# lppllppl920/EndoscopyDepthEstimation-Pytorch

Measured on AMD Instinct MI355X. Metric: train frame-pairs/sec at 256x320 bs=8, higher is better.
Workload: dtype f32

## Files before the change

### endoscopydepthestimation-pytorch_amd/_lib.py

```python

import ctypes
import os

import torch

_HERE = os.path.dirname(os.path.abspath(__file__))
LIB_PATH = os.environ.get("ENDO_HIP_LIB") or os.path.join(_HERE, "lib", "libendo_hip.so")

_P = ctypes.c_void_p
_I = ctypes.c_int
_F = ctypes.c_float
_L = ctypes.c_int64

SIGNATURES = {
    "endo_abi_version": (_I, []),
    "endo_error_string": (ctypes.c_char_p, [_I]),
    "endo_depth_scale_fwd": (_I, [_P, _P, _P, _P, _P, _P, _I, _I, _F, _P]),
    "endo_depth_scale_bwd": (_I, [_P, _P, _P, _P, _P, _P, _P, _I, _I, _F, _P]),
    "endo_flow_from_depth_fwd": (_I, [_P, _P, _P, _P, _P, _P, _I, _I, _I, _P]),
    "endo_flow_from_depth_bwd": (_I, [_P, _P, _P, _P, _P, _P, _P, _I, _I, _I, _P]),
    "endo_depth_warp_fwd": (_I, [_P, _P, _P, _P, _P, _P, _P, _P, _I, _I, _I, _F, _P]),
    "endo_depth_warp_bwd": (_I, [_P, _P, _P, _P, _P, _P, _P, _P, _P, _I, _I, _I, _F, _P]),
    "endo_depth_warp_fwd_tiled": (_I, [_P, _P, _P, _P, _P, _P, _P, _P, _I, _I, _I, _F, _I, _I, _P]),
    "endo_depth_warp_bwd_tiled": (_I, [_P, _P, _P, _P, _P, _P, _P, _P, _P, _I, _I, _I, _F, _I, _I, _P]),
# ... 26 lines not shown
    "endo_net16h_fwd": (_I, [_P, _P, _P, _P, _P, _P, _I, _P]),
    "endo_net16_bwd_workspace_bytes": (_L, [_P]),
    "endo_net16h_bwd_workspace_bytes": (_L, [_P]),
    "endo_net16_set_wgrad_overlap": (_I, [_P, _I]),
    "endo_net16h_set_wgrad_overlap": (_I, [_P, _I]),
    "endo_net16_offset": (_L, [_P, _I, _I]),
    "endo_net16h_offset": (_L, [_P, _I, _I]),
    "endo_net16_bwd": (_I, [_P, _P, _P, _P, _P, _P, _I, _P]),
    "endo_net16h_bwd": (_I, [_P, _P, _P, _P, _P, _P, _I, _P]),
    "endo_mask_mul": (_I, [_P, _P, _P, _I, _I, _I, _P]),
    "endo_net_create": (_I, [ctypes.POINTER(_P), _I, _I, _I]),
    "endo_net_create_grouped": (_I, [ctypes.POINTER(_P), _I, _I, _I, _I]),
    "endo_net_groups": (_I, [_P]),
    "endo_net_set_option": (_I, [_P, _I, _I]),
    "endo_net_get_option": (_I, [_P, _I]),
    "endo_net_group_stride": (_L, [_P]),
    "endo_net_destroy": (None, [_P]),
    "endo_net_param_floats": (_L, []),
    "endo_net_bn_floats": (_L, []),
    "endo_net_tape_floats": (_L, [_P]),
    "endo_net_gradws_floats": (_L, [_P]),
    "endo_net_param_offset": (_L, [_I]),
    "endo_net_bn_offset": (_L, [_I, _I]),
    "endo_net_level_channels": (_I, [_I]),
    "endo_net_act_offset": (_L, [_P, _I]),
    "endo_net_tape_offset": (_L, [_P, _I, _I]),
    "endo_net_fwd": (_I, [_P, _P, _P, _P, _P, _P, _I, _P]),
    "endo_net_bwd": (_I, [_P, _P, _P, _P, _P, _P, _P, _I, _P]),
    "endo_sgd_clip_step": (_I, [_P, _P, _P, _P, _L, _F, _F, _F, _F, _I, _P, _P]),
    "endo_sparse_scatter": (_I, [_P, _I, _P, _P, _P, _P, _P, _I, _I, _I, _F, _P, _P, _P, _P, _P, _P]),
# ... 70 lines not shown
```

### endoscopydepthestimation-pytorch_amd/csrc/net.hip

```cpp
#include <new>
#include <vector>

#include "dgrad_kernels.h"
#include "dgrad_block_kernels.h"
#include "dgrad_newmap_kernels.h"
#include "td_dgrad_kernels.h"
#include "td_fwd_kernels.h"
#include "wgrad_taps_kernels.h"
#include "wgrad1x1_kernels.h"
#include "wgrad_nsplit_kernels.h"
#include "wgrad_x3_kernels.h"
#include "wgrad_f34_kernels.h"
#include "wgrad_subpix_kernels.h"
#include "wino_fwd_kernels.h"
#include "wino4_fwd_kernels.h"
#include "dgrad_wino_kernels.h"
#include "dgrad_wino3_kernels.h"


namespace endo {

int run_dgrad_wino3_nl4(const DgradBlockParams& p, const float* const* u, hipStream_t stream);
bool dgrad_wino3p_applies(const DgradBlockParams& p);
int run_dgrad_wino3p_nl4(const DgradBlockParams& p, const float* const* u, int blocks, double* fw_parts, int* blocks_used, hipStream_t stream);

constexpr int kGrowth = 12;
constexpr int kLayers = 4;
constexpr int kFirst = 48;
constexpr int kLevels = 5;
// ... 102 lines not shown

struct endo_net {
    int n, h, w;
    int groups;
    int64_t gs;
    struct Level { int h, w, t; int64_t plane; int64_t act, grad; int64_t sums; int64_t pq; } lv[kLevels + 1];
    int64_t pre_off;
    int64_t saved_off;
    int64_t idx_off[kLevels];
    int64_t sums_off;
    int64_t sums_bytes;
    int64_t tape_floats;
    int64_t partial_off;
    int64_t wino_off;
    int64_t wino4_off;
    int64_t pq_off;
    int64_t pq_floats;
    int64_t scratch_off;
    int64_t scratch_bytes;
    int64_t slot_stride;
    int64_t wg_scratch_off;
    int64_t tuw_scratch_off;
    int64_t wd_off;
    int64_t gplane_off;
    int64_t bias_parts_off;
    int64_t fw_parts_off;
    int64_t bias_parts_floats;
    int64_t gradws_floats;
    hipStream_t wstream;
    hipEvent_t ev_fork, ev_join;
    int opt[ENDO_OPT_COUNT];
};

namespace endo {


constexpr int kBiasPartChannels = 2048;
constexpr int kBiasPartLaunches = 64;
constexpr int kFwPartBlocks = 512;
struct BiasReduceTable {
    int n;
    struct Entry { const float* parts; float* bias; int count; int nparts; } e[kBiasPartLaunches];
};
struct BiasParts {
    BiasReduceTable table;
    int64_t used;
// ... 144 lines not shown
            if (training) {
                const double mean = a.saved[j][go + 2 * c], rstd = a.saved[j][go + 2 * c + 1];
                const double scale = a.gamma[j][c] * rstd;
                const double k = scale * rstd * s2 / count;
                dp += static_cast<double>(static_cast<float>(-k));
                dq += static_cast<double>(static_cast<float>(-scale * s1 / count + k * mean));
            }
        }
        if (training) {
            pq_p[c] += static_cast<float>(dp);
            pq_q[c] += static_cast<float>(dq);
        }
    }
}

__global__ void tu_phase_weights_kernel(const float* __restrict__ w, int cout, int cin, float* __restrict__ out) {
    constexpr int kPhW = 2 * 12 * 16 + 16;
    const int total = 2 * cin * 2 * 12 * 16;
    for (int i = blockIdx.x * blockDim.x + threadIdx.x; i < total; i += gridDim.x * blockDim.x) {
        const int lane16 = i & 15;
        const int slot = (i >> 4) % 12;
        const int t = (i / (16 * 12)) & 1;
        const int ci = (i / (16 * 12 * 2)) % cin;
        const int a = i / (16 * 12 * 2 * cin);
        int ctap, tile;
        if (slot < 3) { ctap = 0; tile = slot; } else if (slot < 9) { ctap = 1; tile = slot - 3; } else { ctap = 2; tile = slot - 9 + 3; }
        const int b = tile / 3, co = (tile % 3) * 16 + lane16;
        float v = 0.f;
        if (co < cout) {
            const float* src = w + (static_cast<int64_t>(co) * cin + ci) * 9;
            const int ky0 = a == 0 ? (t == 0 ? 0 : 1) : (t == 0 ? 0 : 2), ky1 = a == 0 ? (t == 0 ? 0 : 2) : (t == 0 ? 1 : 2);
            int kx0, kx1;
            if (b == 0) { kx0 = ctap == 0 ? 0 : 1; kx1 = ctap == 0 ? 0 : 2; }
            else { kx0 = ctap == 1 ? 0 : 2; kx1 = ctap == 1 ? 1 : 2; }
            for (int ky = ky0; ky <= ky1; ++ky)
                for (int kx = kx0; kx <= kx1; ++kx) v += src[ky * 3 + kx];
        }
        out[(static_cast<int64_t>(a) * cin + ci) * kPhW + (t * 12 + slot) * 16 + lane16] = v;
    }
}

__global__ void tu_subpix_dgrad_weights_kernel(const float* __restrict__ w, int cout, int cin, float* __restrict__ out) {
    const int pitch = 4 * cin + 16;
    const int total = 4 * cout * 4 * cin;
    for (int i = blockIdx.x * blockDim.x + threadIdx.x; i < total; i += gridDim.x * blockDim.x) {
        const int ci = i % cin;
        const int tap = (i / cin) & 3;
        const int co = (i / (4 * cin)) % cout;
        const int ph = i / (4 * cin * cout);
        const int alpha = ph >> 1, beta = ph & 1, tyi = tap >> 1, txi = tap & 1;
        const int ky0 = alpha == 0 ? (tyi == 0 ? 1 : 0) : (tyi == 0 ? 2 : 0), ky1 = alpha == 0 ? (tyi == 0 ? 2 : 0) : (tyi == 0 ? 2 : 1);
        const int kx0 = beta == 0 ? (txi == 0 ? 1 : 0) : (txi == 0 ? 2 : 0), kx1 = beta == 0 ? (txi == 0 ? 2 : 0) : (txi == 0 ? 2 : 1);
        const float* src = w + (static_cast<int64_t>(co) * cin + ci) * 9;
        float v = 0.f;
// ... 118 lines not shown
        const float t = static_cast<float>(scratch[0] + scratch[1] + scratch[2] + scratch[3]);
        if (c < cin) atomicAdd(gw + c, t); else atomicAdd(gb, t);
    }
}

__global__ void __launch_bounds__(64) final_w_reduce_kernel(const double* __restrict__ parts, int nblocks, int count, float* __restrict__ gw) {
    const int c = blockIdx.x;
    double t = 0.0;
    for (int b = threadIdx.x; b < nblocks; b += 64) t += parts[static_cast<int64_t>(b) * count + c];
    t = wave_sum(t);
    if (threadIdx.x == 0) atomicAdd(gw + c, static_cast<float>(t));
}

constexpr int kBlocks = 2 * kLevels + 1, kDense = kBlocks * kLayers;

enum class DenseFwd { Wino4, Wino2_32x16, Wino2_32x8, SplitK, Direct32x8, Direct16x8, DirectAuto };
struct FwdPlan {
    struct Dense {
        DenseFwd form;
        int stages;
        int ksplit;
        bool chunk_weights;
    } dense[kDense];
    bool bf16;
    bool wino4_weights;
    bool fuse_final;
    bool td_persistent[kLevels];
    bool tu_subpix[kLevels];
};

enum class NewMap { Bf16, Persistent, Vec16, Dword };
// ... 102 lines not shown
static double conv_flops(const endo_net* net, int level, int cin, int cout, int ks) {
    return 2.0 * net->n * net->groups * net->lv[level].plane * cin * cout * ks * ks;
}

static void default_options(int (&opt)[ENDO_OPT_COUNT]) {
    opt[ENDO_OPT_WINO_FWD] = 5;
    opt[ENDO_OPT_WINO_DGRAD] = 3;
    opt[ENDO_OPT_DGRAD_VEC] = 2;
    opt[ENDO_OPT_WINO_MIN_TILES] = 1024;
    opt[ENDO_OPT_MFMA_BF16] = 0;
    opt[ENDO_OPT_WGRAD_OVERLAP] = 1;
    opt[ENDO_OPT_MFMA_X3] = 0;
    opt[ENDO_OPT_WGRAD_F34] = 1;
    opt[ENDO_OPT_FINAL_VIRTUAL] = 1;
    opt[ENDO_OPT_TD_PERSIST] = 3;
}
static int bf16_mask(const int* opt) { const int v = opt[ENDO_OPT_MFMA_BF16]; return v == 1 ? 7 : (v >> 1); }

struct DenseBlock { int level, ic0, c0; const BnP* bn; const ConvP* cv; bool base_overwrite; };
static DenseBlock dense_block(int b) {
    const Table& tb = table();
    if (b < kLevels) return {b, 48, down_in(b), tb.down_bn[b], tb.down_conv[b], false};
    if (b == kLevels) return {kLevels, 0, 288, tb.bott_bn, tb.bott_conv, true};
    const int i = b - kLevels - 1, l = kLevels - 1 - i;
    return {l, 0, 96 + down_in(l), tb.up_bn[i], tb.up_conv[i], l > 0};
}
static long tile_count(const Ctx& c, int level, int tx, int ty) {
    const auto& lv = c.net->lv[level];
    return static_cast<long>((lv.w + tx - 1) / tx) * ((lv.h + ty - 1) / ty) * c.nt();
}
// ... 18 lines not shown
    const ConvP& cv = table().td_conv[level];
    const int next = level + 1;
    const int oc0 = next < kLevels ? 48 : 0;
    ConvParams p{};
    fill_grid(c, p, level);
    fill_in(c, p, c.act(level), level, 48, cv.cin);
    fill_bn_in(c, p, b, level, 48);
    p.wgt = c.params + cv.w; p.bias = c.params + cv.b; p.w_cout = cv.cout; p.w_cin = cv.cin;
    fill_out(c, p, c.act(next), next, oc0, cv.cout);
    p.out_idx = c.idx(level);
    p.idx_ns = static_cast<int64_t>(cv.cout) * c.net->lv[next].plane;
    p.out_sums = c.out_sums(next, oc0);
    return p;
}

static FwdPlan plan_fwd(const Ctx& c) {
    const int* opt = c.net->opt;
    const int mode = opt[ENDO_OPT_WINO_FWD];
    const long min_tiles = opt[ENDO_OPT_WINO_MIN_TILES];
    FwdPlan pl{};
    pl.bf16 = (bf16_mask(opt) & 2) != 0;
    pl.wino4_weights = !pl.bf16 && mode == 5;
    for (int b = 0; b < kBlocks; ++b) {
        const DenseBlock k = dense_block(b);
        const long t64x16 = tile_count(c, k.level, 64, 16), t32x16 = tile_count(c, k.level, 32, 16), t32x8 = tile_count(c, k.level, 32, 8);
        const long t16x16 = tile_count(c, k.level, 16, 16), t16x8 = tile_count(c, k.level, 16, 8);
        const bool big = t32x16 >= min_tiles, small = t32x8 >= (min_tiles * 3) / 4;
        const bool wino4_tiles = mode == 5 && !pl.bf16 && 2 * t64x16 >= min_tiles;
        const bool wino2_tiles = mode != 0 && !pl.bf16 && (big || small);
        for (int j = 0; j < kLayers; ++j) {
            FwdPlan::Dense& d = pl.dense[b * kLayers + j];
            const int nchunks = (k.cv[j].cin + 15) / 16;
            d.chunk_weights = !pl.bf16 && !wino4_tiles && !wino2_tiles;
            d.stages = mode == 4 ? 4 : (mode == 3 ? 3 : 2);
            if (wino4_tiles && wino4_fwd_ok(dense_fwd_params(c, k, j, DenseFwd::Wino4))) {
                d.form = DenseFwd::Wino4;
            } else if (wino2_tiles && wino_fwd_ok(dense_fwd_params(c, k, j, DenseFwd::Wino2_32x16))) {
                d.form = big ? DenseFwd::Wino2_32x16 : DenseFwd::Wino2_32x8;
            } else if (t32x16 < 512 && t16x16 < 384 && t16x8 < 512 && nchunks >= 4) {
                int want = static_cast<int>(((t16x8 < 256 ? 512 : 768) + t16x8 - 1) / t16x8);
                if (want > nchunks) want = nchunks;
                const int per = (nchunks + want - 1) / want;
                d.form = DenseFwd::SplitK;
                d.ksplit = (nchunks + per - 1) / per;
            } else {
                d.form = (t32x16 < 1024 && t32x8 >= 1024) ? DenseFwd::Direct32x8
                       : (t32x16 < 1024 && t16x8 >= 768) ? DenseFwd::Direct16x8 : DenseFwd::DirectAuto;
            }
        }
    }
    pl.fuse_final = opt[ENDO_OPT_FINAL_VIRTUAL] && pl.dense[kDense - 1].form == DenseFwd::Wino4;
    for (int l = 0; l < kLevels; ++l) {
        pl.td_persistent[l] = (opt[ENDO_OPT_TD_PERSIST] & 2) && !pl.bf16 && c.training && td_fwd_ok(td_fwd_params(c, l));
        const ConvP& tu = table().tu_conv[kLevels - 1 - l];
        pl.tu_subpix[l] = c.net->lv[l + 1].w % 4 == 0 && tu.cout == kNew && tu.cin % 4 == 0;
    }
    return pl;
}

// ... 22 lines not shown
            p.split_stride = static_cast<int64_t>(c.net->n) * cv.cout * lv.plane;
            p.out = partial; p.out_ns = static_cast<int64_t>(cv.cout) * lv.plane;
            p.bias = nullptr; p.out_sums = nullptr;
            p.wgt_chunks = chunk_weights;
            int rc = bf16 ? launch_conv_dma<3, 16, 1, IN_BNRELU, EPI_FWD, 1, 2, 2, 1, 1>(p, c.stream)
                          : launch_conv_dma<3, 16, 1, IN_BNRELU, EPI_FWD, 1, 2, 2, 1>(p, c.stream);
            if (rc) return rc;
            int bx = static_cast<int>((lv.plane + 255) / 256);
            bx = bx > 8 ? 8 : bx;
            finalize_partial_kernel<<<dim3(bx, cv.cout, c.nt()), 256, 0, c.stream>>>(
                partial, p.split_stride, d.ksplit, p.out_ns, static_cast<int>(lv.plane), c.params + cv.b, c.act(k.level) + oc0 * lv.plane,
                lv.t * lv.plane, c.out_sums(k.level, oc0), c.net->n, c.net->gs);
            ENDO_LAUNCH_CHECK();
            return 0;
        }
        case DenseFwd::Direct32x8:
            return bf16 ? launch_conv_dma<3, 4, 1, IN_BNRELU, EPI_FWD, 2, 4, 2, 1, 1>(p, c.stream) : launch_conv_dma<3, 4, 1, IN_BNRELU, EPI_FWD, 2, 4, 2, 1>(p, c.stream);
        case DenseFwd::Direct16x8:
            return bf16 ? launch_conv_dma<3, 8, 1, IN_BNRELU, EPI_FWD, 1, 2, 2, 1, 1>(p, c.stream) : launch_conv_dma<3, 8, 1, IN_BNRELU, EPI_FWD, 1, 2, 2, 1>(p, c.stream);
        case DenseFwd::DirectAuto:
            if (bf16) return launch_conv_dma_auto<3, 4, 1, IN_BNRELU, EPI_FWD, 8, 2, 1, 1>(p, c.stream);
            p.wgt_chunks = chunk_weights;
            return launch_conv_dma_auto<3, 4, 1, IN_BNRELU, EPI_FWD, 8, 2, 1>(p, c.stream);
    }
    return ENDO_E_BADARG;
}

static int td_fwd(const Ctx& c, int level) {
    const ConvP& cv = table().td_conv[level];
    const ConvParams p = td_fwd_params(c, level);
    ProfScope prof(kProfConv1x1Pool, c.stream, conv_flops(c.net, level, cv.cin, cv.cout, 1),
                   4.0 * c.nt() * c.net->lv[level].plane * (cv.cin + cv.cout / 4.0));
    if (c.fwd->td_persistent[level]) return launch_td_fwd(p, device_cu_count(), c.stream);
    if (c.fwd->bf16) return launch_conv_dma_auto<1, 8, 3, IN_BNRELU, EPI_FWD_POOL, 4, 2, 1, 1>(p, c.stream);
    return launch_conv_dma_auto<1, 8, 3, IN_BNRELU, EPI_FWD_POOL, 4>(p, c.stream);
}

static int tu_fwd(const Ctx& c, int level, int src_level, int src_c0, const ConvP& cv) {
    ProfScope prof(kProfConv3x3Up, c.stream, conv_flops(c.net, level, cv.cin, cv.cout, 3),
                   4.0 * c.nt() * c.net->lv[level].plane * (cv.cin / 4.0 + cv.cout));
    if (c.fwd->tu_subpix[level]) {
        float* w3 = c.tape + c.net->partial_off;
        tu_phase_weights_kernel<<<(2 * cv.cin * 384 + 255) / 256, 256, 0, c.stream>>>(c.params + cv.w, cv.cout, cv.cin, w3);
        ENDO_LAUNCH_CHECK();
        ConvParams p{};
        fill_grid(c, p, src_level);
        fill_in(c, p, c.act(src_level), src_level, src_c0, cv.cin);
        p.wgt = w3; p.w_cout = 2 * cv.cout; p.w_cin = cv.cin;
        p.bias = c.params + cv.b;
        fill_out(c, p, c.act(level), level, 0, cv.cout);
        p.out_sums = c.out_sums(level, 0);
        return launch_conv_dma_vec<3, 4, 6, IN_PLAIN, EPI_FWD, 2, 4, 2, 1, 4, 0, 0, 2>(p, c.stream);
    }
    ConvParams p{};
    fill_grid(c, p, level);
    fill_in(c, p, c.act(src_level), src_level, src_c0, cv.cin);
    p.wgt = c.params + cv.w; p.bias = c.params + cv.b; p.w_cout = cv.cout; p.w_cin = cv.cin;
    fill_out(c, p, c.act(level), level, 0, cv.cout);
    p.out_sums = c.out_sums(level, 0);
// ... 452 lines not shown

static int64_t align_up(int64_t v, int64_t a) { return (v + a - 1) / a * a; }

}

extern "C" int endo_net_create_grouped(endo_net** out, int n, int h, int w, int groups) {
    if (!out || n <= 0 || h <= 0 || w <= 0 || groups <= 0) return ENDO_E_BADARG;
    if (groups > kMaxGroups) return ENDO_E_UNSUPPORTED;
    if ((h % 32) != 0 || (w % 32) != 0) return ENDO_E_UNSUPPORTED;
    const Table& tb = table();
    endo_net* net = new (std::nothrow) endo_net();
    if (!net) return ENDO_E_BADARG;
    net->n = n; net->h = h; net->w = w; net->groups = groups;
    net->wstream = nullptr; net->ev_fork = nullptr; net->ev_join = nullptr;
    default_options(net->opt);
    int64_t off = 0, sums = 0, pq = 0;
    for (int l = 0; l <= kLevels; ++l) {
        auto& lv = net->lv[l];
        lv.h = h >> l; lv.w = w >> l; lv.t = level_channels(l);
        lv.plane = static_cast<int64_t>(lv.h) * lv.w;
        lv.act = off; lv.grad = off;
        off += align_up(static_cast<int64_t>(n) * lv.t * lv.plane, 64);
        lv.sums = sums; sums += 2 * lv.t;
        lv.pq = pq; pq += lv.t;
    }
    const int64_t acts = off;
    net->pre_off = off; off += align_up(static_cast<int64_t>(n) * h * w, 64);
    net->saved_off = off; off += align_up(2 * tb.bn_width_total, 64);
    int64_t byte_off = off * 4;
    for (int l = 0; l < kLevels; ++l) {
        net->idx_off[l] = byte_off;
        byte_off += align_up(static_cast<int64_t>(n) * (down_in(l) + kNew) * net->lv[l + 1].plane, 256);
    }
    net->sums_off = byte_off;
    net->sums_bytes = sums * 8;
    byte_off += align_up(net->sums_bytes, 256);
    net->partial_off = byte_off / 4;
    byte_off += static_cast<int64_t>(kGrowth) * 163840 * 4;
    net->wino_off = byte_off / 4;
    byte_off += align_up(tb.wino_floats * 4, 256);
    net->wino4_off = byte_off / 4;
    byte_off += align_up(tb.wino4_floats * 4, 256);
    net->tape_floats = byte_off / 4;
    net->pq_off = acts;
    net->pq_floats = 2 * pq;
    net->scratch_off = align_up((acts + net->pq_floats) * 4, 256);
    net->slot_stride = align_up(tb.bn_width_total * 2, 32);
    net->scratch_bytes = net->slot_stride * 8 * kBnSlots;
    net->wg_scratch_off = (net->scratch_off + align_up(net->scratch_bytes, 256)) / 4;
    net->tuw_scratch_off = net->wg_scratch_off + std::max(std::max(kNsScratchFloats, kSpScratchFloats), 4 * kF34ScratchFloats);
    net->wd_off = align_up(net->tuw_scratch_off + 4 * kNew * (4 * kNew + 16), 64);
    net->gplane_off = align_up(net->wd_off + tb.wino_dgrad_floats, 64);
    net->bias_parts_off = net->gplane_off + align_up(static_cast<int64_t>(n) * h * w, 64);
    net->bias_parts_floats = static_cast<int64_t>(kBiasPartChannels) * n * groups * 32;
    {
        int launches = 1, channels = tb.first.cout;
        for (int l = 0; l < kLevels; ++l) {
// ... 24 lines not shown
    return net->opt[option_id];
}

extern "C" void endo_net_destroy(endo_net* net) {
    if (!net) return;
    if (net->ev_fork) (void)hipEventDestroy(net->ev_fork);
    if (net->ev_join) (void)hipEventDestroy(net->ev_join);
    if (net->wstream) (void)hipStreamDestroy(net->wstream);
    delete net;
}
extern "C" int64_t endo_net_param_floats(void) { return table().param_floats; }
extern "C" int64_t endo_net_bn_floats(void) { return table().bn_floats; }
extern "C" int64_t endo_net_tape_floats(const endo_net* net) { return !net ? 0 : (net->groups > 1 ? net->groups * net->gs : net->tape_floats); }
extern "C" int64_t endo_net_gradws_floats(const endo_net* net) { return !net ? 0 : (net->groups > 1 ? net->groups * net->gs : net->gradws_floats); }
extern "C" int endo_net_groups(const endo_net* net) { return net ? net->groups : 0; }
extern "C" int64_t endo_net_group_stride(const endo_net* net) { return net ? net->gs : 0; }
extern "C" int64_t endo_net_param_offset(int index) {
    const Table& tb = table();
    if (index < 0 || index >= static_cast<int>(tb.param_offsets.size())) return -1;
    return tb.param_offsets[index];
}
extern "C" int64_t endo_net_bn_offset(int bn_index, int which) {
    const Table& tb = table();
    if (bn_index < 0 || bn_index >= static_cast<int>(tb.bn_order.size()) || which < 0 || which > 1) return -1;
    return tb.bn_order[bn_index]->run + which * tb.bn_order[bn_index]->c;
}
extern "C" int endo_net_level_channels(int level) { return (level < 0 || level > kLevels) ? -1 : level_channels(level); }
extern "C" int64_t endo_net_act_offset(const endo_net* net, int level) { return (!net || level < 0 || level > kLevels) ? -1 : net->lv[level].act; }

extern "C" int64_t endo_net_tape_offset(const endo_net* net, int what, int index) {
// ... 8 lines not shown
            if (index < 0 || index >= kLevels) return -1;
            return net->idx_off[index];
        default: return -1;
    }
}

extern "C" int endo_net_fwd(endo_net* net, const float* params, float* bn_running, const float* x, float* out, float* tape,
                            int training, void* stream_) {
    if (!net || !params || !bn_running || !x || !out || !tape) return ENDO_E_BADARG;
    const Table& tb = table();
    Ctx c{net, params, bn_running, tape, nullptr, nullptr, training, static_cast<hipStream_t>(stream_)};
    const FwdPlan plan = plan_fwd(c);
    c.fwd = &plan;
    for (int g = 0; g < net->groups; ++g)
        ENDO_CHECK(hipMemsetAsync(reinterpret_cast<char*>(tape + g * net->gs) + net->sums_off, 0, net->sums_bytes, c.stream));
    if (!plan.bf16) {
        ProfScope prof(kProfSmall, c.stream, 0.0, 4.0 * (tb.wino_floats + tb.wino_floats * 9 / 16));
        WinoWeightTable wt = tb.wino;
        for (int l = 0; l < wt.layers; ++l) wt.mode[l] = plan.dense[l].chunk_weights ? 1 : 0;
        wino_fwd_weights_kernel<<<(wt.start[wt.layers] + 255) / 256, 256, 0, c.stream>>>(wt, params, tape + net->wino_off);
        ENDO_LAUNCH_CHECK();
        if (plan.wino4_weights) wino4_fwd_weights_kernel<<<(tb.wino4.start[tb.wino4.layers] + 255) / 256, 256, 0, c.stream>>>(tb.wino4, params, tape + net->wino4_off);
        ENDO_LAUNCH_CHECK();
    }
    int rc;
    {
        ConvParams p{};
        fill_grid(c, p, 0);
        p.in = x; p.in_ns = 3 * net->lv[0].plane; p.in_cs = static_cast<int>(net->lv[0].plane); p.in_w = net->w; p.cin = 3;
        p.in_gs = net->n * p.in_ns;
        p.wgt = params + tb.first.w; p.bias = params + tb.first.b; p.w_cout = kFirst; p.w_cin = 3;
        fill_out(c, p, c.act(0), 0, 48, kFirst);
        p.out_sums = c.out_sums(0, 48);
        ProfScope prof(kProfConvFirst, c.stream, conv_flops(net, 0, 3, kFirst, 3), 4.0 * c.nt() * net->lv[0].plane * (3 + kFirst));
        rc = launch_conv_dma_auto<3, 4, 3, IN_PLAIN, EPI_FWD>(p, c.stream);
        if (rc) return rc;
// ... 134 lines not shown
```

### endoscopydepthestimation-pytorch_amd/csrc/wino_fwd_kernels.h

```cpp
#pragma once

#include "conv_dma_kernels.h"

namespace endo {

constexpr int kWinoUStride = 16 * 16 + 16;
constexpr int kWinoMaxLayers = 48;

struct WinoWeightTable {
    int layers;
    int start[kWinoMaxLayers + 1];
    int cin[kWinoMaxLayers];
    int cout[kWinoMaxLayers];
    int64_t w_off[kWinoMaxLayers];
    int64_t u_off[kWinoMaxLayers];
    int mode[kWinoMaxLayers];
};
constexpr int kDenseChunkFloats = 9 * 16 * 16;

__global__ void __launch_bounds__(256) wino_fwd_weights_kernel(const WinoWeightTable t, const float* __restrict__ params, float* __restrict__ u) {
    const int total = t.start[t.layers];
    for (int item = blockIdx.x * blockDim.x + threadIdx.x; item < total; item += gridDim.x * blockDim.x) {
        int l = 0;
        while (item >= t.start[l + 1]) ++l;
        const int e = item - t.start[l];
        const int ci = e >> 4, j = e & 15;
        float g[3][3];
#pragma unroll
        for (int a = 0; a < 3; ++a)
#pragma unroll
            for (int b = 0; b < 3; ++b) g[a][b] = 0.f;
        if (j < t.cout[l]) {
            const float* src = params + t.w_off[l] + (static_cast<int64_t>(j) * t.cin[l] + ci) * 9;
#pragma unroll
            for (int a = 0; a < 3; ++a)
#pragma unroll
                for (int b = 0; b < 3; ++b) g[a][b] = src[a * 3 + b];
        }
        if (t.mode[l] == 1) {
            float* dst = u + t.u_off[l] + static_cast<int64_t>(ci >> 4) * kDenseChunkFloats + (ci & 15) * 16 + j;
#pragma unroll
            for (int tap = 0; tap < 9; ++tap) dst[tap * 256] = g[tap / 3][tap % 3];
            if (ci == t.cin[l] - 1)
                for (int cz = (ci & 15) + 1; cz < 16; ++cz)
#pragma unroll
                    for (int tap = 0; tap < 9; ++tap) dst[tap * 256 + (cz - (ci & 15)) * 16] = 0.f;
            continue;
        }
        float h[4][3];
#pragma unroll
        for (int b = 0; b < 3; ++b) {
            h[0][b] = g[0][b];
            h[1][b] = 0.5f * (g[0][b] + g[1][b] + g[2][b]);
            h[2][b] = 0.5f * (g[0][b] - g[1][b] + g[2][b]);
            h[3][b] = g[2][b];
        }
        float* dst = u + t.u_off[l] + static_cast<int64_t>(ci) * kWinoUStride + j;
#pragma unroll
        for (int a = 0; a < 4; ++a) {
            dst[(4 * a + 0) * 16] = h[a][0];
            dst[(4 * a + 1) * 16] = 0.5f * (h[a][0] + h[a][1] + h[a][2]);
            dst[(4 * a + 2) * 16] = 0.5f * (h[a][0] - h[a][1] + h[a][2]);
            dst[(4 * a + 3) * 16] = h[a][2];
        }
        if (j == 0) {
#pragma unroll
            for (int k = 0; k < 16; ++k) dst[256 + k] = 0.f;
        }
    }
}

template <int R, int KC, int NS = 2>
struct WinoFwdGeom {
    static constexpr int kTileX = 32;
    static constexpr int kTileY = 8 * R;
    static constexpr int kLeft = 4;
    static constexpr int kCols = kTileX + 2 * kLeft;
    static constexpr int kRows = kTileY + 2;
    static constexpr int kPlane = kRows * kCols;
    static constexpr int kCS = ((kPlane - 32 + 63) / 64) * 64 + 32;
    static constexpr int kUnits = kCS / 4;
    static constexpr int kPos = (kUnits + kConvThreads - 1) / kConvThreads;
    static constexpr int kUUnits = KC * kWinoUStride / 4;
    static constexpr int kUPos = (kUUnits + kConvThreads - 1) / kConvThreads;
// ... 251 lines not shown
```

### endoscopydepthestimation-pytorch_amd/models.py

```python

import ctypes

import torch
from torch import nn

from . import _lib

GROWTH = 12
LAYERS = 4
FIRST = 48
LEVELS = 5


class ConvParams(nn.Module):

    def __init__(self, cin, cout, k):
        super().__init__()
        self.weight = nn.Parameter(torch.empty(cout, cin, k, k))
        self.bias = nn.Parameter(torch.zeros(cout))
        nn.init.kaiming_uniform_(self.weight, a=5 ** 0.5)


class FusedBatchNorm2d(nn.Module):

# ... 218 lines not shown
                p.grad = self._flat_grad[off:off + p.numel()].view(p.shape)

    def _handle(self, n, h, w, groups=1):
        key = (n, h, w, groups)
        if key not in self._handles:
            lib = _lib.load()
            if lib.endo_net_param_floats() != self._flat.numel():
                raise RuntimeError("parameter packing mismatch between Python and libendo_hip.so")
            hnd = ctypes.c_void_p()
            _lib.check(lib.endo_net_create_grouped(ctypes.byref(hnd), n, h, w, groups), "endo_net_create_grouped(%d,%d,%d,%d)" % key)
            for option_id, value in getattr(self, "_kernel_options", {}).items():
                lib.endo_net_set_option(hnd, option_id, value)
            self._handles[key] = (hnd, int(lib.endo_net_tape_floats(hnd)), int(lib.endo_net_gradws_floats(hnd)))
        return self._handles[key]

    _OPTION_DEFAULTS = {0: 5, 1: 3, 2: 2, 3: 1024, 4: 0, 5: 1, 6: 0, 7: 1, 8: 1, 9: 3}

    def set_kernel_option(self, option_id, value):
        option_id, value = int(option_id), int(value)
        if option_id not in self._OPTION_DEFAULTS:
            raise ValueError("unknown kernel option %d" % option_id)
        options = self.__dict__.setdefault("_kernel_options", {})
        old = options.get(option_id, self._OPTION_DEFAULTS[option_id])
        options[option_id] = value
        lib = _lib.load()
        for key, (hnd, _, _) in self._handles.items():
            if key[0] in ("bf16", "fp16"):
                continue
            rc = lib.endo_net_set_option(hnd, option_id, value)
            if rc < 0:
                raise RuntimeError("endo_net_set_option(%d, %d) failed: %d" % (option_id, value, rc))
# ... 334 lines not shown
```

### include/endo_hip.h

```cpp
#ifndef ENDO_HIP_H
#define ENDO_HIP_H

#include <stdint.h>

#ifdef __cplusplus
extern "C" {
#endif

#define ENDO_E_BADARG (-1)
#define ENDO_E_UNSUPPORTED (-2)

#define ENDO_ABI_VERSION 6
int endo_abi_version(void);
const char* endo_error_string(int code);

int endo_depth_scale_fwd(const float* pred, const float* sparse_depth, const float* sparse_mask,
                         float* scaled, float* ratio, double* stats,
                         int n, int hw, float eps, void* stream);
int endo_depth_scale_bwd(const float* grad_scaled, const float* grad_ratio,
                         const float* pred, const float* sparse_depth, const double* stats,
                         float* grad_pred, double* work,
                         int n, int hw, float eps, void* stream);

int endo_flow_from_depth_fwd(const float* depth, const float* mask, const float* t, const float* R,
// ... 66 lines not shown
typedef struct endo_net endo_net;

int endo_net_create(endo_net** out, int n, int h, int w);
int endo_net_create_grouped(endo_net** out, int n, int h, int w, int groups);
int endo_net_groups(const endo_net* net);
#define ENDO_OPT_WINO_FWD 0
#define ENDO_OPT_WINO_DGRAD 1
#define ENDO_OPT_DGRAD_VEC 2
#define ENDO_OPT_WINO_MIN_TILES 3
#define ENDO_OPT_MFMA_BF16 4
#define ENDO_OPT_WGRAD_OVERLAP 5
#define ENDO_OPT_MFMA_X3 6
#define ENDO_OPT_WGRAD_F34 7
#define ENDO_OPT_FINAL_VIRTUAL 8
#define ENDO_OPT_TD_PERSIST 9
#define ENDO_OPT_COUNT 10
int endo_net_set_option(endo_net* net, int option_id, int value);
int endo_net_get_option(const endo_net* net, int option_id);
int64_t endo_net_group_stride(const endo_net* net);
void endo_net_destroy(endo_net* net);
int64_t endo_net_param_floats(void);
int64_t endo_net_bn_floats(void);
int64_t endo_net_tape_floats(const endo_net* net);
int64_t endo_net_gradws_floats(const endo_net* net);
int64_t endo_net_param_offset(int index);
int64_t endo_net_bn_offset(int bn_index, int which );

int endo_net_fwd(endo_net* net, const float* params, float* bn_running, const float* x, float* out,
                 float* tape, int training, void* stream);
int endo_net_bwd(endo_net* net, const float* params, const float* x, const float* tape,
                 const float* grad_out, float* grads, float* gradws, int training, void* stream);
int endo_net_level_channels(int level);
int64_t endo_net_act_offset(const endo_net* net, int level);
// ... 122 lines not shown
```

Baseline: 512.6.

## Add opt-in block-level k-split conv and fuse forward weight prep launches

Adds a new dense 3x3 forward conv kernel that splits input-channel chunks across wave groups inside one block and reduces the partial sums in LDS, instead of using separate split-K partials. It is gated by a new option that defaults to 0, so it stays off unless enabled. Separately, the transposed-conv phase-weight precomputation moves out of the per-level path into one fused weight-prep launch alongside the Winograd weight transform. That launch now also runs in bf16 mode, and the precomputed weights get their own tape regions. This removes several small kernel launches per step at the cost of extra tape memory.

```diff
diff --git a/endoscopydepthestimation-pytorch_amd/_lib.py b/endoscopydepthestimation-pytorch_amd/_lib.py
--- a/endoscopydepthestimation-pytorch_amd/_lib.py
+++ b/endoscopydepthestimation-pytorch_amd/_lib.py
@@ -64,6 +64,7 @@
     "endo_net_groups": (_I, [_P]),
     "endo_net_set_option": (_I, [_P, _I, _I]),
     "endo_net_get_option": (_I, [_P, _I]),
+    "endo_net_ksplit_block_launches": (_L, [_P]),
     "endo_net_group_stride": (_L, [_P]),
     "endo_net_destroy": (None, [_P]),
     "endo_net_param_floats": (_L, []),
diff --git a/endoscopydepthestimation-pytorch_amd/csrc/conv_ksplit_kernels.h b/endoscopydepthestimation-pytorch_amd/csrc/conv_ksplit_kernels.h
--- /dev/null
+++ b/endoscopydepthestimation-pytorch_amd/csrc/conv_ksplit_kernels.h
@@ -0,0 +1,264 @@
+#pragma once
+
+#include "wino_fwd_kernels.h"
+
+namespace endo {
+
+constexpr int ksplit_max_slices(int ws) { return ws == 4 ? 3 : 4; }
+
+template <int R, int WS, int VEC>
+struct KSplitGeom {
+    static constexpr int kThreads = 64 * WS;
+    static constexpr int kMaxSlices = ksplit_max_slices(WS);
+    static constexpr int kTileX = 16, kTileY = R * WS;
+    static constexpr int kRows = kTileY + 2;
+    static constexpr int kLeft = VEC == 4 ? 4 : 1;
+    static constexpr int kCols = kTileX + 2 * kLeft;
+    static constexpr int kColOff = kLeft - 1;
+    static constexpr int kPlane = kRows * kCols;
+    static constexpr int kCS = ((kPlane - 16 + 31) / 32) * 32 + 16;
+    static constexpr int kUnits = kPlane / VEC;
+    static constexpr int kPos = (kUnits + kThreads - 1) / kThreads;
+    static constexpr int kW = kDenseChunkFloats;
+    static constexpr int kBuf = 16 * kCS + kW;
+    static constexpr int kSlice = 2 * kBuf;
+    static constexpr int kRed = 2 * 16 * WS;
+    static_assert(4 * R * kThreads <= kBuf, "a slice's accumulators fit one of its staging buffers");
+    static_assert(kCS % 4 == 0 && kBuf % 4 == 0, "16-byte DMA destinations");
+    static size_t bytes(int slices, int bn_cap) { return sizeof(float) * (static_cast<size_t>(slices) * kSlice + 3 * bn_cap + kRed); }
+};
+
+constexpr size_t kKSplitLdsLimit = 160 * 1024;
+
+template <int R, int WS, int VEC>
+__global__ void __launch_bounds__(64 * WS * ksplit_max_slices(WS)) conv_ksplit_kernel(const ConvParams p0) {
+    using G = KSplitGeom<R, WS, VEC>;
+    constexpr int KC = 16, KS = 3, NB = 16;
+    constexpr int T = G::kThreads;
+    extern __shared__ __attribute__((aligned(16))) float smem[];
+    const int slices = p0.ksplit;
+    float* s_aux = smem + slices * G::kSlice;
+    float* s_red = s_aux + 3 * p0.bn_cap;
+    int grp, n;
+    group_of(p0, blockIdx.z, grp, n);
+    const ConvParams p = group_view(p0, grp);
+    const int groups = p0.group_n > 0 ? gridDim.z / p0.group_n : 1;
+    const bool first_of_group = blockIdx.x == 0 && n == 0;
+    const int cap = p.bn_cap;
+
+    const int tid = threadIdx.x;
+    const int lane = tid & 63;
+    const int slice = __builtin_amdgcn_readfirstlane(tid / T);
+    const int ts = tid - slice * T;
+    const int wave = __builtin_amdgcn_readfirstlane(ts >> 6);
+    const int tile = (gridDim.x & 7) == 0 ? xcd_remap(blockIdx.x, gridDim.x) : blockIdx.x;
+    const int x0 = (tile % p.tiles_x) * G::kTileX;
+    const int y0 = (tile / p.tiles_x) * G::kTileY;
+    float* s_slice = smem + slice * G::kSlice;
+
+    for (int c = tid; c < p.cin; c += blockDim.x) {
+        float scale, mean, beta;
+        bn_input_constants(p, p0, grp, groups, first_of_group, c, scale, mean, beta);
+        s_aux[c] = scale;
+        s_aux[cap + c] = mean;
+        s_aux[2 * cap + c] = beta;
+    }
+    for (int c = p.cin + tid; c < ((p.cin + KC - 1) / KC) * KC; c += blockDim.x) {
+        s_aux[c] = 0.f; s_aux[cap + c] = 0.f; s_aux[2 * cap + c] = 0.f;
+    }
+
+    f32x4 acc[R];
+#pragma unroll
+    for (int r = 0; r < R; ++r) acc[r] = f32x4{0.f, 0.f, 0.f, 0.f};
+    const int wy = wave * R;
+    const int li = lane & 15;
+    const int lk = lane >> 4;
+
+    int goff[G::kPos];
+    unsigned pos_ok = 0;
+#pragma unroll
+    for (int k = 0; k < G::kPos; ++k) {
+        const int e = ts + k * T;
+        goff[k] = 0;
+        if (e < G::kUnits) {
+            const int ry = e / (G::kCols / VEC);
+            const int rx = (e - ry * (G::kCols / VEC)) * VEC;
+            const int gy = y0 - 1 + ry;
+            const int gx = x0 - G::kLeft + rx;
+            if (gy >= 0 && gy < p.h && gx >= 0 && gx < p.w) {
+                pos_ok |= (1u << k);
+                goff[k] = gy * p.in_w + gx;
+            }
+        }
+    }
+    const float* in_n = p.in + n * p.in_ns;
+    const float* pad_in = g_pad_consts;
+    const int nchunks_all = (p.cin + KC - 1) / KC;
+    const int per = (nchunks_all + slices - 1) / slices;
+    const int chunk_begin = slice * per;
+    const int chunk_end = min(nchunks_all, chunk_begin + per);
+
+    auto issue_dma = [&](int chunk, int buf) {
+        const int c_base = chunk * KC;
+        float* s_in = s_slice + buf * G::kBuf;
+        float* s_w = s_in + KC * G::kCS;
+#pragma unroll
+        for (int c = 0; c < KC; ++c) {
+            const int ch = c_base + c;
+            const float* plane = in_n + static_cast<int64_t>(ch) * p.in_cs;
+#pragma unroll
+            for (int k = 0; k < G::kPos; ++k) {
+                const int e0 = k * T + wave * 64;
+                if (e0 < G::kUnits) {
+                    const bool ok = (ch < p.cin) && (pos_ok & (1u << k));
+                    const float* src = ok ? plane + goff[k] : pad_in;
+                    if (e0 + lane < G::kUnits) {
+                        if constexpr (VEC == 4)
+                            __builtin_amdgcn_global_load_lds((gptr_t)src, (lptr_t)(s_in + c * G::kCS + 4 * e0), 16, 0, 0);
+                        else
+                            __builtin_amdgcn_global_load_lds((gptr_t)src, (lptr_t)(s_in + c * G::kCS + e0), 4, 0, 0);
+                    }
+                }
+            }
+        }
+        constexpr int kUnitsW = G::kW / 4;
+        const float* wsrc = p.wgt_chunks + static_cast<int64_t>(chunk) * G::kW;
+#pragma unroll
+        for (int k = 0; k < (kUnitsW + T - 1) / T; ++k) {
+            const int u0 = k * T + wave * 64;
+            if (u0 < kUnitsW && u0 + lane < kUnitsW)
+                __builtin_amdgcn_global_load_lds((gptr_t)(wsrc + 4 * (u0 + lane)), (lptr_t)(s_w + 4 * u0), 16, 0, 0);
+        }
+    };
+
+    auto compute = [&](int chunk, int buf) {
+        const float* s_in = s_slice + buf * G::kBuf;
+        const float* s_w = s_in + KC * G::kCS;
+        typedef float f32x2 __attribute__((ext_vector_type(2)));
+        constexpr int NR = R + KS - 1;
+#pragma unroll
+        for (int quad = 0; quad < KC / 4; ++quad) {
+            const float* a_base = s_in + (quad * 4 + lk) * G::kCS + wy * G::kCols + li + G::kColOff;
+            const float* b_base = s_w + (quad * 4 + lk) * NB + li;
+            const int ch = chunk * KC + quad * 4 + lk;
+            const float sc = s_aux[ch], mn = s_aux[cap + ch], bt = s_aux[2 * cap + ch];
+            const f32x2 mn2 = {mn, mn}, sc2 = {sc, sc}, bt2 = {bt, bt};
+#pragma unroll
+            for (int dx = 0; dx < KS; ++dx) {
+                float a[NR];
+#pragma unroll
+                for (int r = 0; r + 1 < NR; r += 2) {
+                    f32x2 v = {a_base[r * G::kCols + dx], a_base[(r + 1) * G::kCols + dx]};
+                    v = __builtin_elementwise_fma(v - mn2, sc2, bt2);
+                    a[r] = __builtin_fmaxf(v[0], 0.f);
+                    a[r + 1] = __builtin_fmaxf(v[1], 0.f);
+                }
+                if constexpr (NR & 1) a[NR - 1] = __builtin_fmaxf(fmaf(a_base[(NR - 1) * G::kCols + dx] - mn, sc, bt), 0.f);
+#pragma unroll
+                for (int dy = 0; dy < KS; ++dy) {
+                    const float b = b_base[(dy * KS + dx) * KC * NB];
+#pragma unroll
+                    for (int r = 0; r < R; ++r) acc[r] = __builtin_amdgcn_mfma_f32_16x16x4f32(a[r + dy], b, acc[r], 0, 0, 0);
+                }
+            }
+        }
+    };
+
+    if (chunk_begin < chunk_end) issue_dma(chunk_begin, 0);
+    for (int i = 0; i < per; ++i) {
+        const int chunk = chunk_begin + i;
+        const int b = i & 1;
+        asm volatile("s_waitcnt vmcnt(0)" ::: "memory");
+        __syncthreads();
+        if (chunk + 1 < chunk_end) issue_dma(chunk + 1, b ^ 1);
+        if (chunk < chunk_end) compute(chunk, b);
+    }
+
+    f32x4* s_acc = reinterpret_cast<f32x4*>(s_slice + (per & 1) * G::kBuf);
+    if (slice > 0) {
+#pragma unroll
+        for (int r = 0; r < R; ++r) s_acc[r * T + ts] = acc[r];
+    }
+    __syncthreads();
+    if (slice == 0) {
+        const int px = x0 + 4 * lk;
+        const bool vec_ok = ((p.out_w & 3) == 0) && ((p.w & 3) == 0);
+        const bool co_ok = li < p.cout;
+        const float bias = co_ok ? p.bias[li] : 0.f;
+        float s1 = 0.f, s2 = 0.f;
+#pragma unroll
+        for (int r = 0; r < R; ++r) {
+            const int y = y0 + wy + r;
+            f32x4 v = acc[r];
+            v[0] += bias; v[1] += bias; v[2] += bias; v[3] += bias;
+            for (int s = 1; s < slices; ++s) {
+                const f32x4 o = reinterpret_cast<const f32x4*>(smem + s * G::kSlice + (per & 1) * G::kBuf)[r * T + ts];
+                v[0] += o[0]; v[1] += o[1]; v[2] += o[2]; v[3] += o[3];
+            }
+            if (co_ok && y < p.h) {
+                float* dst = p.out + n * p.out_ns + static_cast<int64_t>(li) * p.out_cs + y * p.out_w + px;
+                if (vec_ok && px + 3 < p.w) {
+                    *reinterpret_cast<f32x4*>(dst) = v;
+#pragma unroll
+                    for (int e = 0; e < 4; ++e) { s1 += v[e]; s2 += v[e] * v[e]; }
+                } else {
+#pragma unroll
+                    for (int e = 0; e < 4; ++e)
+                        if (px + e < p.w) { dst[e] = v[e]; s1 += v[e]; s2 += v[e] * v[e]; }
+                }
+            }
+        }
+        if (p.out_sums) {
+            s1 += __shfl_xor(s1, 16, 64); s1 += __shfl_xor(s1, 32, 64);
+            s2 += __shfl_xor(s2, 16, 64); s2 += __shfl_xor(s2, 32, 64);
+            if (lk == 0) {
+                s_red[(wave * NB + li) * 2] = s1;
+                s_red[(wave * NB + li) * 2 + 1] = s2;
+            }
+        }
+    }
+    if (p.out_sums) {
+        __syncthreads();
+        if (tid < 2 * NB) {
+            const int j = tid >> 1, which = tid & 1;
+            if (j < p.cout) {
+                double t = 0.0;
+                for (int wv = 0; wv < WS; ++wv) t += static_cast<double>(s_red[(wv * NB + j) * 2 + which]);
+                atomicAdd(p.out_sums + 2 * j + which, t);
+            }
+        }
+    }
+}
+
+inline bool conv_ksplit_aligned(const ConvParams& p) {
+    return (p.w % 4 == 0) && (p.in_w % 4 == 0) && (p.in_cs % 4 == 0) && (p.in_ns % 4 == 0) && (reinterpret_cast<uintptr_t>(p.in) % 16 == 0);
+}
+
+template <int R, int WS>
+inline bool conv_ksplit_ok(const ConvParams& p, int slices) {
+    const int nchunks = (p.cin + 15) / 16;
+    if (!p.bias || p.cout > 16 || p.cin > kMaxBnChannels || slices < 1 || slices > nchunks) return false;
+    if (slices > KSplitGeom<R, WS, 4>::kMaxSlices) return false;
+    const int per = (nchunks + slices - 1) / slices;
+    if ((nchunks + per - 1) / per != slices) return false;
+    const int cap = nchunks * 16;
+    return (conv_ksplit_aligned(p) ? KSplitGeom<R, WS, 4>::bytes(slices, cap) : KSplitGeom<R, WS, 1>::bytes(slices, cap)) <= kKSplitLdsLimit;
+}
+
+template <int R, int WS, int VEC>
+inline int launch_conv_ksplit_vec(ConvParams p, int slices, hipStream_t stream) {
+    using G = KSplitGeom<R, WS, VEC>;
+    p.tiles_x = (p.w + G::kTileX - 1) / G::kTileX;
+    p.bn_cap = (p.cin + 15) / 16 * 16;
+    p.ksplit = slices;
+    const int tiles_y = (p.h + G::kTileY - 1) / G::kTileY;
+    return launch_dyn(conv_ksplit_kernel<R, WS, VEC>, dim3(p.tiles_x * tiles_y, 1, p.n), dim3(slices * G::kThreads), G::bytes(slices, p.bn_cap), stream, p);
+}
+
+template <int R, int WS>
+inline int launch_conv_ksplit(const ConvParams& p, int slices, hipStream_t stream) {
+    if (!p.wgt_chunks || !conv_ksplit_ok<R, WS>(p, slices)) return ENDO_E_BADARG;
+    return conv_ksplit_aligned(p) ? launch_conv_ksplit_vec<R, WS, 4>(p, slices, stream) : launch_conv_ksplit_vec<R, WS, 1>(p, slices, stream);
+}
+
+}
diff --git a/endoscopydepthestimation-pytorch_amd/csrc/net.hip b/endoscopydepthestimation-pytorch_amd/csrc/net.hip
--- a/endoscopydepthestimation-pytorch_amd/csrc/net.hip
+++ b/endoscopydepthestimation-pytorch_amd/csrc/net.hip
@@ -13,6 +13,7 @@
 #include "wgrad_f34_kernels.h"
 #include "wgrad_subpix_kernels.h"
 #include "wino_fwd_kernels.h"
+#include "conv_ksplit_kernels.h"
 #include "wino4_fwd_kernels.h"
 #include "dgrad_wino_kernels.h"
 #include "dgrad_wino3_kernels.h"
@@ -145,6 +146,7 @@
     int64_t partial_off;
     int64_t wino_off;
     int64_t wino4_off;
+    int64_t tuw_off[kLevels];
     int64_t pq_off;
     int64_t pq_floats;
     int64_t scratch_off;
@@ -161,6 +163,7 @@
     hipStream_t wstream;
     hipEvent_t ev_fork, ev_join;
     int opt[ENDO_OPT_COUNT];
+    int64_t ksplit_block_launches;
 };
 
 namespace endo {
@@ -335,30 +338,49 @@
     }
 }
 
-__global__ void tu_phase_weights_kernel(const float* __restrict__ w, int cout, int cin, float* __restrict__ out) {
+__device__ __forceinline__ void tu_phase_weights_item(const float* __restrict__ w, int cout, int cin, float* __restrict__ out, int i) {
     constexpr int kPhW = 2 * 12 * 16 + 16;
-    const int total = 2 * cin * 2 * 12 * 16;
-    for (int i = blockIdx.x * blockDim.x + threadIdx.x; i < total; i += gridDim.x * blockDim.x) {
-        const int lane16 = i & 15;
-        const int slot = (i >> 4) % 12;
-        const int t = (i / (16 * 12)) & 1;
-        const int ci = (i / (16 * 12 * 2)) % cin;
-        const int a = i / (16 * 12 * 2 * cin);
-        int ctap, tile;
-        if (slot < 3) { ctap = 0; tile = slot; } else if (slot < 9) { ctap = 1; tile = slot - 3; } else { ctap = 2; tile = slot - 9 + 3; }
-        const int b = tile / 3, co = (tile % 3) * 16 + lane16;
-        float v = 0.f;
-        if (co < cout) {
-            const float* src = w + (static_cast<int64_t>(co) * cin + ci) * 9;
-            const int ky0 = a == 0 ? (t == 0 ? 0 : 1) : (t == 0 ? 0 : 2), ky1 = a == 0 ? (t == 0 ? 0 : 2) : (t == 0 ? 1 : 2);
-            int kx0, kx1;
-            if (b == 0) { kx0 = ctap == 0 ? 0 : 1; kx1 = ctap == 0 ? 0 : 2; }
-            else { kx0 = ctap == 1 ? 0 : 2; kx1 = ctap == 1 ? 1 : 2; }
-            for (int ky = ky0; ky <= ky1; ++ky)
-                for (int kx = kx0; kx <= kx1; ++kx) v += src[ky * 3 + kx];
-        }
-        out[(static_cast<int64_t>(a) * cin + ci) * kPhW + (t * 12 + slot) * 16 + lane16] = v;
-    }
+    const int lane16 = i & 15;
+    const int slot = (i >> 4) % 12;
+    const int t = (i / (16 * 12)) & 1;
+    const int ci = (i / (16 * 12 * 2)) % cin;
+    const int a = i / (16 * 12 * 2 * cin);
+    int ctap, tile;
+    if (slot < 3) { ctap = 0; tile = slot; } else if (slot < 9) { ctap = 1; tile = slot - 3; } else { ctap = 2; tile = slot - 9 + 3; }
+    const int b = tile / 3, co = (tile % 3) * 16 + lane16;
+    float v = 0.f;
+    if (co < cout) {
+        const float* src = w + (static_cast<int64_t>(co) * cin + ci) * 9;
+        const int ky0 = a == 0 ? (t == 0 ? 0 : 1) : (t == 0 ? 0 : 2), ky1 = a == 0 ? (t == 0 ? 0 : 2) : (t == 0 ? 1 : 2);
+        int kx0, kx1;
+        if (b == 0) { kx0 = ctap == 0 ? 0 : 1; kx1 = ctap == 0 ? 0 : 2; }
+        else { kx0 = ctap == 1 ? 0 : 2; kx1 = ctap == 1 ? 1 : 2; }
+        for (int ky = ky0; ky <= ky1; ++ky)
+            for (int kx = kx0; kx <= kx1; ++kx) v += src[ky * 3 + kx];
+    }
+    out[(static_cast<int64_t>(a) * cin + ci) * kPhW + (t * 12 + slot) * 16 + lane16] = v;
+}
+constexpr int64_t tu_phase_floats(int cin) { return 2 * static_cast<int64_t>(cin) * 400; }
+
+struct TuPhaseTable {
+    int count;
+    int start[kLevels + 1];
+    int cin[kLevels], cout[kLevels];
+    int64_t w_off[kLevels];
+    int64_t out_off[kLevels];
+};
+__global__ void __launch_bounds__(256) fwd_weights_kernel(const WinoWeightTable t, const float* __restrict__ params, float* __restrict__ u, int wino_blocks,
+                                                          const TuPhaseTable tu, float* __restrict__ tape) {
+    if (static_cast<int>(blockIdx.x) < wino_blocks) {
+        const int item = blockIdx.x * 256 + threadIdx.x;
+        if (item < t.start[t.layers]) wino_fwd_weights_item(t, params, u, item);
+        return;
+    }
+    const int item = (blockIdx.x - wino_blocks) * 256 + threadIdx.x;
+    if (item >= tu.start[tu.count]) return;
+    int l = 0;
+    while (item >= tu.start[l + 1]) ++l;
+    tu_phase_weights_item(params + tu.w_off[l], tu.cout[l], tu.cin[l], tape + tu.out_off[l], item - tu.start[l]);
 }
 
 __global__ void tu_subpix_dgrad_weights_kernel(const float* __restrict__ w, int cout, int cin, float* __restrict__ out) {
@@ -507,7 +529,7 @@
 
 constexpr int kBlocks = 2 * kLevels + 1, kDense = kBlocks * kLayers;
 
-enum class DenseFwd { Wino4, Wino2_32x16, Wino2_32x8, SplitK, Direct32x8, Direct16x8, DirectAuto };
+enum class DenseFwd { Wino4, Wino2_32x16, Wino2_32x8, SplitK, KSplitBlock16x8, KSplitBlock16x4, Direct32x8, Direct16x8, DirectAuto };
 struct FwdPlan {
     struct Dense {
         DenseFwd form;
@@ -640,6 +662,7 @@
     opt[ENDO_OPT_WGRAD_F34] = 1;
     opt[ENDO_OPT_FINAL_VIRTUAL] = 1;
     opt[ENDO_OPT_TD_PERSIST] = 3;
+    opt[ENDO_OPT_KSPLIT_BLOCK] = 0;
 }
 static int bf16_mask(const int* opt) { const int v = opt[ENDO_OPT_MFMA_BF16]; return v == 1 ? 7 : (v >> 1); }
 
@@ -688,6 +711,7 @@
     return p;
 }
 
+constexpr int kKSplitBlockAdopted = 3;
 static FwdPlan plan_fwd(const Ctx& c) {
     const int* opt = c.net->opt;
     const int mode = opt[ENDO_OPT_WINO_FWD];
@@ -695,6 +719,7 @@
     FwdPlan pl{};
     pl.bf16 = (bf16_mask(opt) & 2) != 0;
     pl.wino4_weights = !pl.bf16 && mode == 5;
+    const int ksplit_block = opt[ENDO_OPT_KSPLIT_BLOCK] == 1 ? kKSplitBlockAdopted : (opt[ENDO_OPT_KSPLIT_BLOCK] >> 1);
     for (int b = 0; b < kBlocks; ++b) {
         const DenseBlock k = dense_block(b);
         const long t64x16 = tile_count(c, k.level, 64, 16), t32x16 = tile_count(c, k.level, 32, 16), t32x8 = tile_count(c, k.level, 32, 8);
@@ -717,6 +742,16 @@
                 const int per = (nchunks + want - 1) / want;
                 d.form = DenseFwd::SplitK;
                 d.ksplit = (nchunks + per - 1) / per;
+                if (ksplit_block && !pl.bf16 && d.chunk_weights) {
+                    const ConvParams p = dense_fwd_params(c, k, j, DenseFwd::SplitK);
+                    const int s4 = nchunks < 4 ? nchunks : 4, per4 = (nchunks + s4 - 1) / s4, slices4 = (nchunks + per4 - 1) / per4;
+                    if ((ksplit_block & 1) && d.ksplit <= 3 && conv_ksplit_ok<2, 4>(p, d.ksplit)) {
+                        d.form = DenseFwd::KSplitBlock16x8;
+                    } else if ((ksplit_block & 2) && d.ksplit > 3 && tile_count(c, k.level, 16, 4) <= 256 && conv_ksplit_ok<2, 2>(p, slices4)) {
+                        d.form = DenseFwd::KSplitBlock16x4;
+                        d.ksplit = slices4;
+                    }
+                }
             } else {
                 d.form = (t32x16 < 1024 && t32x8 >= 1024) ? DenseFwd::Direct32x8
                        : (t32x16 < 1024 && t16x8 >= 768) ? DenseFwd::Direct16x8 : DenseFwd::DirectAuto;
@@ -769,6 +804,11 @@
             ENDO_LAUNCH_CHECK();
             return 0;
         }
+        case DenseFwd::KSplitBlock16x8:
+        case DenseFwd::KSplitBlock16x4:
+            p.wgt_chunks = chunk_weights;
+            ++const_cast<endo_net*>(c.net)->ksplit_block_launches;
+            return d.form == DenseFwd::KSplitBlock16x8 ? launch_conv_ksplit<2, 4>(p, d.ksplit, c.stream) : launch_conv_ksplit<2, 2>(p, d.ksplit, c.stream);
         case DenseFwd::Direct32x8:
             return bf16 ? launch_conv_dma<3, 4, 1, IN_BNRELU, EPI_FWD, 2, 4, 2, 1, 1>(p, c.stream) : launch_conv_dma<3, 4, 1, IN_BNRELU, EPI_FWD, 2, 4, 2, 1>(p, c.stream);
         case DenseFwd::Direct16x8:
@@ -795,9 +835,7 @@
     ProfScope prof(kProfConv3x3Up, c.stream, conv_flops(c.net, level, cv.cin, cv.cout, 3),
                    4.0 * c.nt() * c.net->lv[level].plane * (cv.cin / 4.0 + cv.cout));
     if (c.fwd->tu_subpix[level]) {
-        float* w3 = c.tape + c.net->partial_off;
-        tu_phase_weights_kernel<<<(2 * cv.cin * 384 + 255) / 256, 256, 0, c.stream>>>(c.params + cv.w, cv.cout, cv.cin, w3);
-        ENDO_LAUNCH_CHECK();
+        const float* w3 = c.tape + c.net->tuw_off[kLevels - 1 - level];
         ConvParams p{};
         fill_grid(c, p, src_level);
         fill_in(c, p, c.act(src_level), src_level, src_c0, cv.cin);
@@ -1280,6 +1318,7 @@
     net->n = n; net->h = h; net->w = w; net->groups = groups;
     net->wstream = nullptr; net->ev_fork = nullptr; net->ev_join = nullptr;
     default_options(net->opt);
+    net->ksplit_block_launches = 0;
     int64_t off = 0, sums = 0, pq = 0;
     for (int l = 0; l <= kLevels; ++l) {
         auto& lv = net->lv[l];
@@ -1307,6 +1346,10 @@
     byte_off += align_up(tb.wino_floats * 4, 256);
     net->wino4_off = byte_off / 4;
     byte_off += align_up(tb.wino4_floats * 4, 256);
+    for (int i = 0; i < kLevels; ++i) {
+        net->tuw_off[i] = byte_off / 4;
+        byte_off += align_up(tu_phase_floats(tb.tu_conv[i].cin) * 4, 256);
+    }
     net->tape_floats = byte_off / 4;
     net->pq_off = acts;
     net->pq_floats = 2 * pq;
@@ -1361,6 +1404,7 @@
 extern "C" int64_t endo_net_tape_floats(const endo_net* net) { return !net ? 0 : (net->groups > 1 ? net->groups * net->gs : net->tape_floats); }
 extern "C" int64_t endo_net_gradws_floats(const endo_net* net) { return !net ? 0 : (net->groups > 1 ? net->groups * net->gs : net->gradws_floats); }
 extern "C" int endo_net_groups(const endo_net* net) { return net ? net->groups : 0; }
+extern "C" int64_t endo_net_ksplit_block_launches(const endo_net* net) { return net ? net->ksplit_block_launches : -1; }
 extern "C" int64_t endo_net_group_stride(const endo_net* net) { return net ? net->gs : 0; }
 extern "C" int64_t endo_net_param_offset(int index) {
     const Table& tb = table();
@@ -1399,12 +1443,25 @@
     c.fwd = &plan;
     for (int g = 0; g < net->groups; ++g)
         ENDO_CHECK(hipMemsetAsync(reinterpret_cast<char*>(tape + g * net->gs) + net->sums_off, 0, net->sums_bytes, c.stream));
-    if (!plan.bf16) {
+    {
         ProfScope prof(kProfSmall, c.stream, 0.0, 4.0 * (tb.wino_floats + tb.wino_floats * 9 / 16));
         WinoWeightTable wt = tb.wino;
         for (int l = 0; l < wt.layers; ++l) wt.mode[l] = plan.dense[l].chunk_weights ? 1 : 0;
-        wino_fwd_weights_kernel<<<(wt.start[wt.layers] + 255) / 256, 256, 0, c.stream>>>(wt, params, tape + net->wino_off);
+        if (plan.bf16) wt.layers = 0;
+        const int wino_blocks = (wt.start[wt.layers] + 255) / 256;
+        TuPhaseTable tu{};
+        for (int i = 0; i < kLevels; ++i) {
+            if (!plan.tu_subpix[kLevels - 1 - i]) continue;
+            const ConvP& cv = tb.tu_conv[i];
+            tu.cin[tu.count] = cv.cin; tu.cout[tu.count] = cv.cout; tu.w_off[tu.count] = cv.w; tu.out_off[tu.count] = net->tuw_off[i];
+            tu.start[tu.count + 1] = tu.start[tu.count] + 2 * cv.cin * 384;
+            ++tu.count;
+        }
+        const int blocks = wino_blocks + (tu.start[tu.count] + 255) / 256;
+        if (blocks > 0) fwd_weights_kernel<<<blocks, 256, 0, c.stream>>>(wt, params, tape + net->wino_off, wino_blocks, tu, tape);
         ENDO_LAUNCH_CHECK();
+    }
+    if (!plan.bf16) {
         if (plan.wino4_weights) wino4_fwd_weights_kernel<<<(tb.wino4.start[tb.wino4.layers] + 255) / 256, 256, 0, c.stream>>>(tb.wino4, params, tape + net->wino4_off);
         ENDO_LAUNCH_CHECK();
     }
diff --git a/endoscopydepthestimation-pytorch_amd/csrc/wino_fwd_kernels.h b/endoscopydepthestimation-pytorch_amd/csrc/wino_fwd_kernels.h
--- a/endoscopydepthestimation-pytorch_amd/csrc/wino_fwd_kernels.h
+++ b/endoscopydepthestimation-pytorch_amd/csrc/wino_fwd_kernels.h
@@ -18,9 +18,8 @@
 };
 constexpr int kDenseChunkFloats = 9 * 16 * 16;
 
-__global__ void __launch_bounds__(256) wino_fwd_weights_kernel(const WinoWeightTable t, const float* __restrict__ params, float* __restrict__ u) {
-    const int total = t.start[t.layers];
-    for (int item = blockIdx.x * blockDim.x + threadIdx.x; item < total; item += gridDim.x * blockDim.x) {
+__device__ __forceinline__ void wino_fwd_weights_item(const WinoWeightTable& t, const float* __restrict__ params, float* __restrict__ u, int item) {
+    {
         int l = 0;
         while (item >= t.start[l + 1]) ++l;
         const int e = item - t.start[l];
@@ -45,7 +44,7 @@
                 for (int cz = (ci & 15) + 1; cz < 16; ++cz)
 #pragma unroll
                     for (int tap = 0; tap < 9; ++tap) dst[tap * 256 + (cz - (ci & 15)) * 16] = 0.f;
-            continue;
+            return;
         }
         float h[4][3];
 #pragma unroll
@@ -68,6 +67,11 @@
             for (int k = 0; k < 16; ++k) dst[256 + k] = 0.f;
         }
     }
+}
+
+__global__ void __launch_bounds__(256) wino_fwd_weights_kernel(const WinoWeightTable t, const float* __restrict__ params, float* __restrict__ u) {
+    const int total = t.start[t.layers];
+    for (int item = blockIdx.x * blockDim.x + threadIdx.x; item < total; item += gridDim.x * blockDim.x) wino_fwd_weights_item(t, params, u, item);
 }
 
 template <int R, int KC, int NS = 2>
diff --git a/endoscopydepthestimation-pytorch_amd/models.py b/endoscopydepthestimation-pytorch_amd/models.py
--- a/endoscopydepthestimation-pytorch_amd/models.py
+++ b/endoscopydepthestimation-pytorch_amd/models.py
@@ -256,7 +256,7 @@
             self._handles[key] = (hnd, int(lib.endo_net_tape_floats(hnd)), int(lib.endo_net_gradws_floats(hnd)))
         return self._handles[key]
 
-    _OPTION_DEFAULTS = {0: 5, 1: 3, 2: 2, 3: 1024, 4: 0, 5: 1, 6: 0, 7: 1, 8: 1, 9: 3}
+    _OPTION_DEFAULTS = {0: 5, 1: 3, 2: 2, 3: 1024, 4: 0, 5: 1, 6: 0, 7: 1, 8: 1, 9: 3, 10: 0}
 
     def set_kernel_option(self, option_id, value):
         option_id, value = int(option_id), int(value)
diff --git a/include/endo_hip.h b/include/endo_hip.h
--- a/include/endo_hip.h
+++ b/include/endo_hip.h
@@ -104,9 +104,11 @@
 #define ENDO_OPT_WGRAD_F34 7
 #define ENDO_OPT_FINAL_VIRTUAL 8
 #define ENDO_OPT_TD_PERSIST 9
-#define ENDO_OPT_COUNT 10
+#define ENDO_OPT_KSPLIT_BLOCK 10
+#define ENDO_OPT_COUNT 11
 int endo_net_set_option(endo_net* net, int option_id, int value);
 int endo_net_get_option(const endo_net* net, int option_id);
+int64_t endo_net_ksplit_block_launches(const endo_net* net);
 int64_t endo_net_group_stride(const endo_net* net);
 void endo_net_destroy(endo_net* net);
 int64_t endo_net_param_floats(void);
```

Result: no change. 513.2, median of 4 (+0.1%).
